# Xiaoming-Zhao/PointNav-VO

Hardware: AMD Instinct MI355X
Metric: RGB-D frame-pair VO inferences/s @341x192 (higher is better)
Workload: dtype f32

## Files before the change

pointnav-vo_amd/csrc/conv_x3.hip:

```cpp
#include <cmath>
#include <cstdio>
#include <cstdlib>
#include <cstring>

#include "pnvo_internal.h"

namespace pnvo {

typedef float f32x16 __attribute__((ext_vector_type(16)));
typedef float f32x4 __attribute__((ext_vector_type(4)));
typedef float f32x2 __attribute__((ext_vector_type(2)));
typedef __bf16 bf16x8 __attribute__((ext_vector_type(8)));
typedef __bf16 bf16x2 __attribute__((ext_vector_type(2)));
typedef _Float16 f16x8 __attribute__((ext_vector_type(8)));
typedef _Float16 f16x2 __attribute__((ext_vector_type(2)));
typedef unsigned u32x4 __attribute__((ext_vector_type(4)));

namespace {
__device__ __forceinline__ unsigned pack2(float a, float b) {
  const bf16x2 r = __builtin_convertvector(f32x2{a, b}, bf16x2);
  return __builtin_bit_cast(unsigned, r);
}
__device__ __forceinline__ unsigned pack2h(float a, float b) {
  const f16x2 r = __builtin_convertvector(f32x2{a, b}, f16x2);
  return __builtin_bit_cast(unsigned, r);
}
__device__ __forceinline__ float lo_f(unsigned u) { return __builtin_bit_cast(float, u << 16); }
__device__ __forceinline__ float hi_f(unsigned u) { return __builtin_bit_cast(float, u & 0xffff0000u); }
}

constexpr int x3_wpe(int mw, int nw, int np, bool dsf = false) {
  return dsf ? (mw * nw >= 6 ? 1 : (mw * nw >= 2 ? 2 : 3)) : ((np == 2 && mw * nw <= 2) ? 3 : 2);
}

template <int KS, int STRIDE, int MODE, int MW, int NW, int NP, bool DSF = false, bool W8 = false, bool KSW = false>
__global__ __launch_bounds__(W8 ? 512 : 256) __attribute__((amdgpu_waves_per_eu(W8 ? 2 : x3_wpe(MW, NW, NP, DSF), W8 ? 2 : x3_wpe(MW, NW, NP, DSF)))) void conv_x3_kernel(const ConvX3Args p) {
  constexpr int NTH = W8 ? 512 : 256, NWV = NTH / 64;
  constexpr int EMW = KSW ? 1 : MW;
  static_assert(!KSW || (NW == 1 && NP == 2 && KS == 3 && !DSF && !W8), "K split over the waves: float16-piece 3x3 convs, one N-tile");
  static_assert(!DSF || (KS == 3 && STRIDE == 2 && NP == 2 && (MODE == 0 || MODE == 2)), "the downsample rides on a float16-piece 3x3 stride-2 conv");
  extern __shared__ __attribute__((aligned(16))) unsigned char lds[];
  constexpr int PSTEP = KS == 1 ? STRIDE : 1;
  constexpr int CS = KS == 1 ? 1 : STRIDE;
  constexpr int PAD = KS / 2;
  const int lane = threadIdx.x & 63;
  const int wave = __builtin_amdgcn_readfirstlane(threadIdx.x >> 6);

  const int ntiles = p.B * p.tiles_r * p.tiles_c;
  const int chunk = (ntiles + 7) >> 3;
  int bid = (int)(blockIdx.x & 7) * chunk + (int)(blockIdx.x >> 3);
  if (bid >= ntiles) return;
  const int tci = bid % p.tiles_c;
  bid /= p.tiles_c;
  const int tri = bid % p.tiles_r;
  const int n = bid / p.tiles_r;
  const int r0 = tri * p.TR, c0 = tci * p.TC;
  const int hi0 = r0 * STRIDE - PAD, wi0 = c0 * STRIDE - PAD;
  const int mdl = (p.grp_end0 > 0 && n >= p.grp_end0) + (p.grp_end1 > 0 && n >= p.grp_end1);
  const unsigned short *g_wpk = mdl == 0 ? p.wpk : p.wpk_g[mdl - 1];
  const unsigned short *g_ds_wpk = mdl == 0 ? p.ds_wpk : p.ds_wpk_g[mdl - 1];
  const float g_oscale = mdl == 0 ? p.oscale : p.oscale_g[mdl - 1], g_ds_oscale = mdl == 0 ? p.ds_oscale : p.ds_oscale_g[mdl - 1];
  const float *g_gamma = mdl == 0 ? p.gn_gamma : p.gn_gamma_g[mdl - 1], *g_beta = mdl == 0 ? p.gn_beta : p.gn_beta_g[mdl - 1];
  const float *g_ds_gamma = mdl == 0 ? p.ds_gamma : p.ds_gamma_g[mdl - 1], *g_ds_beta = mdl == 0 ? p.ds_beta : p.ds_beta_g[mdl - 1];
  const int PR = p.PR, PC = p.PC, CK = p.CK;
  const int pitch = CK * 2 + 16;
  const int plane = PR * PC * pitch;
  const int npix = p.TR * p.TC;
  const int tab_off = KSW ? max(NP * plane, 4 * MW * 4096) : NP * plane;
  unsigned *qtab = reinterpret_cast<unsigned *>(lds + tab_off);
  unsigned *otab = qtab + p.MT * 32;
  for (int e = (int)threadIdx.x; e < p.MT * 32; e += NTH) {
    const int q = min(e, npix - 1);
    const int tr = q / p.TC, tc = q - tr * p.TC;
    qtab[e] = (unsigned)(((tr * CS) * PC + tc * CS) * pitch);
    const bool ok = e < npix && r0 + tr < p.Ho && c0 + tc < p.Wo;
    otab[e] = (unsigned)((tr * p.Wo + tc) * p.COUTP) | (ok ? 0u : 0x80000000u);
  }

  const int wn = p.wn;
  const int wave_m = wave / wn;
  const int wave_n = (wave & (wn - 1)) + (int)blockIdx.y * wn;
  const int ntt = p.COUTP >> 5, kct = p.CIN >> 4;

  f32x16 acc[MW][NW];
#pragma unroll
  for (int i = 0; i < MW; ++i)
#pragma unroll
    for (int j = 0; j < NW; ++j)
#pragma unroll
      for (int r = 0; r < 16; ++r) acc[i][j][r] = 0.f;
  f32x16 accd[DSF ? MW : 1][DSF ? NW : 1];
  if (DSF) {
#pragma unroll
    for (int i = 0; i < MW; ++i)
#pragma unroll
      for (int j = 0; j < NW; ++j)
#pragma unroll
        for (int r = 0; r < 16; ++r) accd[DSF ? i : 0][DSF ? j : 0][r] = 0.f;
  }

  float in_mul = 1.f, in_div = 1.f;
  const bool in_scaled = NP == 2 && p.in_absmax != nullptr;
  if (in_scaled) {
    unsigned mb = p.in_absmax[(threadIdx.x & 63) * 16];
#pragma unroll
    for (int d = 32; d >= 1; d >>= 1) mb = max(mb, (unsigned)__shfl_xor((int)mb, d));
    const int e = mb != 0u ? (int)((mb >> 23) & 0xffu) - 126 : 14;
    in_mul = __builtin_bit_cast(float, (unsigned)(14 - e + 127) << 23);
    in_div = __builtin_bit_cast(float, (unsigned)(e - 14 + 127) << 23);
  }
  const int G = CK >> 3;
  const int cg = threadIdx.x & (G - 1), pl = threadIdx.x / G, PS = NTH / G;
  const int dr = PS / PC, dc = PS - dr * PC;
  const int nppix = PR * PC;

  unsigned long long c_stage = 0, c_mm = 0, t_0 = __builtin_readcyclecounter(), r_0 = wall_clock64();
  for (int ck0 = 0; ck0 < p.CIN; ck0 += CK) {
    unsigned long long t_a = __builtin_readcyclecounter();
    if (ck0 > 0) __syncthreads();
    {
      f32x4 sc0, sc1, sh0, sh1, rs0, rs1, rt0, rt1;
      const bool res_ss = MODE == 2 && p.res_scale != nullptr;
      auto load_ss = [&]() {
        if (MODE >= 1) {
          const float *ps = p.in_scale + (long)n * p.CIN + ck0 + 8 * cg;
          const float *pt = p.in_shift + (long)n * p.CIN + ck0 + 8 * cg;
          sc0 = *reinterpret_cast<const f32x4 *>(ps);
          sc1 = *reinterpret_cast<const f32x4 *>(ps + 4);
          sh0 = *reinterpret_cast<const f32x4 *>(pt);
          sh1 = *reinterpret_cast<const f32x4 *>(pt + 4);
        }
        if (res_ss) {
          const float *ps = p.res_scale + (long)n * p.CIN + ck0 + 8 * cg;
          const float *pt = p.res_shift + (long)n * p.CIN + ck0 + 8 * cg;
          rs0 = *reinterpret_cast<const f32x4 *>(ps);
          rs1 = *reinterpret_cast<const f32x4 *>(ps + 4);
          rt0 = *reinterpret_cast<const f32x4 *>(pt);
          rt1 = *reinterpret_cast<const f32x4 *>(pt + 4);
        }
      };
      load_ss();
      int pr = pl / PC, pc = pl - pr * PC;
      const long img = ((long)n * p.H * p.W) * p.CIN + ck0 + 8 * cg;
      const float *xb = p.x + img;
      struct Round {
        f32x4 v[2][2], w[2][2];
        unsigned off[2];
        int gofs[2];
        bool ok[2], in[2], own[2];
      };
      auto fetch = [&](int pix, Round &r) {
#pragma unroll
        for (int k = 0; k < 2; ++k) {
          const int hi = hi0 + pr * PSTEP, wi = wi0 + pc * PSTEP;
          r.ok[k] = pix + k * PS < nppix;
          r.in[k] = r.ok[k] && hi >= 0 && hi < p.H && wi >= 0 && wi < p.W;
          r.off[k] = (unsigned)((pr * PC + pc) * pitch + 16 * cg);
          r.v[k][0] = r.v[k][1] = f32x4{0.f, 0.f, 0.f, 0.f};
          if (MODE >= 2) {
            r.own[k] = r.in[k] && p.xout != nullptr && blockIdx.y == 0 && pr >= PAD && pr < PAD + p.TR * CS && pc >= PAD && pc < PAD + p.TC * CS;
            r.gofs[k] = (hi * p.W + wi) * p.CIN;
          }
          if (r.in[k]) {
            const float *src = xb + ((long)hi * p.W + wi) * p.CIN;
            r.v[k][0] = *reinterpret_cast<const f32x4 *>(src);
            r.v[k][1] = *reinterpret_cast<const f32x4 *>(src + 4);
            if (MODE == 2) {
              const float *rsrc = p.res + img + ((long)hi * p.W + wi) * p.CIN;
              r.w[k][0] = *reinterpret_cast<const f32x4 *>(rsrc);
              r.w[k][1] = *reinterpret_cast<const f32x4 *>(rsrc + 4);
            }
          }
          pr += dr;
          pc += dc;
          if (pc >= PC) {
            pc -= PC;
            pr += 1;
          }
        }
      };
      auto split_store = [&](const Round &r) {
#pragma unroll
        for (int k = 0; k < 2; ++k) {
          if (!r.ok[k]) continue;
          float f[8];
#pragma unroll
          for (int e = 0; e < 8; ++e) {
            float t = r.v[k][e >> 2][e & 3];
            if (MODE == 1) {
              const f32x4 &sc = e < 4 ? sc0 : sc1, &sh = e < 4 ? sh0 : sh1;
              t = r.in[k] ? fmaxf(__builtin_fmaf(t, sc[e & 3], sh[e & 3]), 0.f) : 0.f;
            }
            if (MODE == 3) {
              const f32x4 &sc = e < 4 ? sc0 : sc1, &sh = e < 4 ? sh0 : sh1;
              int key = __builtin_bit_cast(int, t);
              key = key >= 0 ? key : key ^ 0x7fffffff;
              t = r.in[k] ? fmaxf(__builtin_fmaf(__builtin_bit_cast(float, key), __builtin_fabsf(sc[e & 3]), sh[e & 3]), 0.f) : 0.f;
            }
            if (MODE == 2) {
              const f32x4 &sc = e < 4 ? sc0 : sc1, &sh = e < 4 ? sh0 : sh1;
              float u = r.w[k][e >> 2][e & 3];
              if (res_ss) u = __builtin_fmaf(u, (e < 4 ? rs0 : rs1)[e & 3], (e < 4 ? rt0 : rt1)[e & 3]);
              t = r.in[k] ? fmaxf(__builtin_fmaf(t, sc[e & 3], sh[e & 3]) + u, 0.f) : 0.f;
            }
            f[e] = t;
          }
          if (MODE >= 2 && r.own[k]) {
            float *dst = p.xout + img + r.gofs[k];
            *reinterpret_cast<f32x4 *>(dst) = f32x4{f[0], f[1], f[2], f[3]};
            *reinterpret_cast<f32x4 *>(dst + 4) = f32x4{f[4], f[5], f[6], f[7]};
          }
          if (NP == 2) {
            if (in_scaled) {
#pragma unroll
              for (int e = 0; e < 8; ++e) f[e] *= in_mul;
            }
            u32x4 o0, o1;
#pragma unroll
            for (int e = 0; e < 4; ++e) {
              const float a = f[2 * e], b = f[2 * e + 1];
              const f16x2 h = __builtin_convertvector(f32x2{a, b}, f16x2);
              o0[e] = __builtin_bit_cast(unsigned, h);
              o1[e] = pack2h(a - (float)h[0], b - (float)h[1]);
            }
            *reinterpret_cast<u32x4 *>(lds + r.off[k]) = o0;
            *reinterpret_cast<u32x4 *>(lds + plane + r.off[k]) = o1;
            continue;
          }
          u32x4 o0, o1, o2;
#pragma unroll
          for (int e = 0; e < 4; ++e) {
            const float a = f[2 * e], b = f[2 * e + 1];
            const unsigned h = pack2(a, b);
            const float ra = a - lo_f(h), rb = b - hi_f(h);
            const unsigned m = pack2(ra, rb);
            o0[e] = h;
            o1[e] = m;
            o2[e] = pack2(ra - lo_f(m), rb - hi_f(m));
          }
          *reinterpret_cast<u32x4 *>(lds + r.off[k]) = o0;
          *reinterpret_cast<u32x4 *>(lds + plane + r.off[k]) = o1;
          *reinterpret_cast<u32x4 *>(lds + 2 * plane + r.off[k]) = o2;
        }
      };
      constexpr bool PIPE = !((MODE == 2 && (MW * NW >= 6 || x3_wpe(MW, NW, NP) == 3 || DSF)) || (DSF && MW * NW == 4));
      if (MW * NW <= 2 && !(MODE == 2 && (x3_wpe(MW, NW, NP) == 3 || DSF))) {
        for (int pix = pl; pix < nppix; pix += 6 * PS) {
          Round r0, r1, r2;
          fetch(pix, r0);
          fetch(pix + 2 * PS, r1);
          fetch(pix + 4 * PS, r2);
          split_store(r0);
          split_store(r1);
          split_store(r2);
        }
      } else if (PIPE) {
        Round cur, nxt;
        fetch(pl, cur);
        for (int pix = pl; pix < nppix; pix += 2 * PS) {
          const bool more = pix + 2 * PS < nppix;
          if (more) fetch(pix + 2 * PS, nxt);
          split_store(cur);
          if (more) cur = nxt;
        }
      } else {
        for (int pix = pl; pix < nppix; pix += 2 * PS) {
          Round cur;
          fetch(pix, cur);
          split_store(cur);
        }
      }
    }
    __syncthreads();
    unsigned long long t_b = __builtin_readcyclecounter();
    c_stage += t_b - t_a;

    unsigned aoff[MW];
#pragma unroll
    for (int i = 0; i < MW; ++i) {
      const int mt = min(KSW ? i : wave_m * MW + i, p.MT - 1);
      aoff[i] = qtab[mt * 32 + (lane & 31)] + (unsigned)((lane >> 5) * 16);
    }
    const int kcc = CK >> 4;
    const int nsteps = KS * KS * kcc;
    const unsigned kstep = (unsigned)ntt * (NP * 1024u);
    const char *wb_n = reinterpret_cast<const char *>(g_wpk) + (long)(ck0 >> 4) * kstep;
    unsigned toff_n = 0;
    int kc_n = 0, kw_n = 0;
    auto advance = [&]() {
      ++kc_n;
      toff_n += 32;
      wb_n += kstep;
      if (kc_n == kcc) {
        kc_n = 0;
        toff_n += (unsigned)(pitch - kcc * 32);
        wb_n += (long)(kct - kcc) * kstep;
        if (++kw_n == KS) {
          kw_n = 0;
          toff_n += (unsigned)((PC - KS) * pitch);
        }
      }
    };
    constexpr bool RING = NP == 2 && KS == 3 && MW * NW <= 2;
    const char *wb_b = wb_n;
    int kc_b = 0;
    auto advanceB = [&]() {
      wb_b += kstep;
      if (++kc_b == kcc) {
        kc_b = 0;
        wb_b += (long)(kct - kcc) * kstep;
      }
    };
    unsigned voff[NW];
#pragma unroll
    for (int j = 0; j < NW; ++j) voff[j] = (unsigned)min(wave_n * NW + j, ntt - 1) * (NP * 1024u) + (unsigned)lane * 16u;
    auto loadBr = [&](u32x4 (*b)[NW]) {
#pragma unroll
      for (int j = 0; j < NW; ++j)
#pragma unroll
        for (int pc = 0; pc < NP; ++pc) b[pc][j] = *reinterpret_cast<const u32x4 *>(wb_b + (size_t)voff[j] + pc * 1024);
    };
    auto loadA = [&](int i, u32x4 (*a)[MW]) {
#pragma unroll
      for (int pc = 0; pc < NP; ++pc) a[pc][i] = *reinterpret_cast<const u32x4 *>(lds + pc * plane + aoff[i] + toff_n);
    };
    auto loadB = [&](u32x4 (*b)[NW]) {
#pragma unroll
      for (int j = 0; j < NW; ++j)
#pragma unroll
        for (int pc = 0; pc < NP; ++pc) b[pc][j] = *reinterpret_cast<const u32x4 *>(wb_n + (size_t)voff[j] + pc * 1024);
    };
    auto step = [&](u32x4 (*a)[MW], const u32x4 (*b)[NW]) {
#pragma unroll
      for (int i = 0; i < MW; ++i) {
#pragma unroll
        for (int j = 0; j < NW; ++j) {
          if (NP == 2) {
            constexpr int TA[3] = {1, 0, 0}, TB[3] = {0, 1, 0};
#pragma unroll
            for (int t = 0; t < 3; ++t)
              acc[i][j] = __builtin_amdgcn_mfma_f32_32x32x16_f16(__builtin_bit_cast(f16x8, a[TA[t]][i]),
                                                                 __builtin_bit_cast(f16x8, b[TB[t]][j]), acc[i][j], 0, 0, 0);
          } else {
            constexpr int TA[6] = {1, 2, 0, 1, 0, 0}, TB[6] = {1, 0, 2, 0, 1, 0};
#pragma unroll
            for (int t = 0; t < 6; ++t)
              acc[i][j] = __builtin_amdgcn_mfma_f32_32x32x16_bf16(__builtin_bit_cast(bf16x8, a[TA[t]][i]),
                                                                  __builtin_bit_cast(bf16x8, b[TB[t]][j]), acc[i][j], 0, 0, 0);
          }
        }
        __builtin_amdgcn_sched_barrier(0);
        loadA(i, a);
        __builtin_amdgcn_sched_barrier(0);
      }
    };
    u32x4 a[NP][MW], b0[NP][NW], b1[NP][NW];
    u32x4 bd0[DSF ? NP : 1][NW], bd1[DSF ? NP : 1][NW];
    auto loadBd = [&](u32x4 (*b)[NW], int kc) {
      const char *wd = reinterpret_cast<const char *>(g_ds_wpk) + (long)((ck0 >> 4) + kc) * kstep;
#pragma unroll
      for (int j = 0; j < NW; ++j)
#pragma unroll
        for (int pc = 0; pc < NP; ++pc) b[pc][j] = *reinterpret_cast<const u32x4 *>(wd + (size_t)voff[j] + pc * 1024);
    };
    if constexpr (KSW) {
      const int s0 = (wave * nsteps) >> 2, s1 = ((wave + 1) * nsteps) >> 2;
      {
        const int tap = s0 / kcc, kc = s0 - tap * kcc, kh = tap / KS, kw = tap - kh * KS;
        kc_n = kc;
        kw_n = kw;
        toff_n = (unsigned)((kh * PC + kw) * pitch + kc * 32);
        wb_n += ((long)tap * kct + kc) * kstep;
        kc_b = kc;
        wb_b = wb_n;
      }
      u32x4 br[3][NP][NW];
      int fb = s0;
      auto fetchB = [&](u32x4 (*bq)[NW]) {
        loadBr(bq);
        if (++fb < s1) advanceB();
      };
      fetchB(br[0]);
      fetchB(br[1]);
#pragma unroll
      for (int i = 0; i < MW; ++i) loadA(i, a);
      if (s0 + 1 < s1) advance();
#pragma unroll 1
      for (int s = s0; s < s1; s += 3) {
#pragma unroll
        for (int u = 0; u < 3; ++u) {
          if (s + u >= s1) break;
          fetchB(br[(u + 2) % 3]);
          __builtin_amdgcn_sched_barrier(0);
          step(a, br[u]);
          if (s + u + 2 < s1) advance();
        }
      }
    } else {
    if (DSF) loadBd(bd0, 0);
    loadB(b0);
#pragma unroll
    for (int i = 0; i < MW; ++i) loadA(i, a);
    advance();
    if (RING) {
      constexpr int R = MW * NW <= 2 ? 6 : 3;
      u32x4 br[R][NP][NW];
#pragma unroll
      for (int pc = 0; pc < NP; ++pc)
#pragma unroll
        for (int j = 0; j < NW; ++j) br[0][pc][j] = b0[pc][j];
#pragma unroll
      for (int q = 1; q < R - 1; ++q) {
        advanceB();
        loadBr(br[q]);
      }
      advanceB();
      constexpr bool A2 = MW * NW <= 2 && !(MODE == 2 && MW * NW == 2 && !DSF) && !(MODE == 2 && DSF && MW * NW == 1);
      u32x4 a1[A2 ? NP : 1][MW];
      if (A2) {
#pragma unroll
        for (int i = 0; i < MW; ++i) loadA(i, a1);
        advance();
      }
#pragma unroll 1
      for (int s = 0; s < nsteps; s += R) {
#pragma unroll
        for (int u = 0; u < R; ++u) {
          loadBr(br[(u + R - 1) % R]);
          if (s + u + R < nsteps) advanceB();
          __builtin_amdgcn_sched_barrier(0);
          if (A2) {
            step((u & 1) ? a1 : a, br[u]);
            if (s + u + 3 < nsteps) advance();
          } else {
            step(a, br[u]);
            if (s + u + 2 < nsteps) advance();
          }
        }
      }
    } else {
#pragma unroll 1
      for (int s = 0; s < nsteps; s += 2) {
        const bool more = s + 2 < nsteps;
        loadB(b1);
        __builtin_amdgcn_sched_barrier(0);
        step(a, b0);
        if (more) advance();
        loadB(b0);
        __builtin_amdgcn_sched_barrier(0);
        step(a, b1);
        if (more) advance();
      }
    }
    }
    if constexpr (DSF) {
      const unsigned tc0 = (unsigned)((PC + 1) * pitch);
      u32x4 ad[NP][MW];
      auto loadAd = [&](int kc) {
#pragma unroll
        for (int i = 0; i < MW; ++i)
#pragma unroll
          for (int pc = 0; pc < NP; ++pc) ad[pc][i] = *reinterpret_cast<const u32x4 *>(lds + pc * plane + aoff[i] + tc0 + (unsigned)kc * 32u);
      };
      auto mm = [&](const u32x4 (*bd)[NW]) {
        constexpr int TA[3] = {1, 0, 0}, TB[3] = {0, 1, 0};
#pragma unroll
        for (int i = 0; i < MW; ++i)
#pragma unroll
          for (int j = 0; j < NW; ++j)
#pragma unroll
            for (int t = 0; t < 3; ++t)
              accd[i][j] = __builtin_amdgcn_mfma_f32_32x32x16_f16(__builtin_bit_cast(f16x8, ad[TA[t]][i]), __builtin_bit_cast(f16x8, bd[TB[t]][j]),
                                                                  accd[i][j], 0, 0, 0);
      };
      if constexpr (MW * NW == 4) {
#pragma unroll 1
        for (int kc = 0; kc < kcc; ++kc) {
          loadAd(kc);
          mm(bd0);
          if (kc + 1 < kcc) loadBd(bd0, kc + 1);
        }
      } else {
#pragma unroll 1
        for (int kc = 0; kc < kcc; kc += 2) {
          loadAd(kc);
          loadBd(bd1, kc + 1);
          mm(bd0);
          loadAd(kc + 1);
          if (kc + 2 < kcc) loadBd(bd0, kc + 2);
          mm(bd1);
        }
      }
    }
    c_mm += __builtin_readcyclecounter() - t_b;
  }
  if constexpr (KSW) {
    __syncthreads();
    float *part = reinterpret_cast<float *>(lds);
#pragma unroll
    for (int i = 0; i < MW; ++i)
#pragma unroll
      for (int r = 0; r < 16; ++r) part[((wave * MW + i) * 16 + r) * 64 + lane] = acc[i][0][r];
    __syncthreads();
    const int mt = min(wave, MW - 1);
#pragma unroll
    for (int r = 0; r < 16; ++r) {
      float v = part[((0 * MW + mt) * 16 + r) * 64 + lane];
#pragma unroll
      for (int w = 1; w < 4; ++w) v += part[((w * MW + mt) * 16 + r) * 64 + lane];
      acc[0][0][r] = v;
    }
    __syncthreads();
  }
  unsigned long long t_e = __builtin_readcyclecounter();

  const int rr16 = lane >> 5;
  const long ybase = (((long)n * p.Ho + r0) * p.Wo + c0) * p.COUTP;
  auto emit = [&](f32x16 (*ac)[NW], float *yout, float *stats, const float *oscale_ptr, float oscale, const float *gamma, const float *beta,
                  float *gscale, float *gshift, float *gmu, float *grstd, bool again) {
    if (NP == 2) {
      const float os = (oscale_ptr != nullptr ? *oscale_ptr : oscale) * in_div;
#pragma unroll
      for (int i = 0; i < EMW; ++i)
#pragma unroll
        for (int j = 0; j < NW; ++j)
#pragma unroll
          for (int r = 0; r < 16; ++r) ac[i][j][r] *= os;
    }
    float t1[NW], t2[NW];
#pragma unroll
    for (int j = 0; j < NW; ++j) t1[j] = t2[j] = 0.f;
#pragma unroll
    for (int i = 0; i < EMW; ++i) {
      const int mt = KSW ? wave : wave_m * MW + i;
      if (mt >= p.MT) continue;
      u32x4 ent[4];
#pragma unroll
      for (int g4 = 0; g4 < 4; ++g4) ent[g4] = *reinterpret_cast<const u32x4 *>(otab + mt * 32 + 8 * g4 + 4 * rr16);
      unsigned flags = 0;
#pragma unroll
      for (int g4 = 0; g4 < 4; ++g4) flags |= ent[g4][0] | ent[g4][1] | ent[g4][2] | ent[g4][3];
      const bool whole = !__any((int)(flags >> 31));
#pragma unroll
      for (int j = 0; j < NW; ++j) {
        const int nt = wave_n * NW + j;
        if (nt >= ntt) continue;
        const int co = nt * 32 + (lane & 31);
        float s1 = 0.f, s2 = 0.f;
        if (whole) {
#pragma unroll
          for (int r = 0; r < 16; ++r) {
            const float v = ac[i][j][r];
            (yout + ybase + co)[ent[r >> 2][r & 3]] = v;
            s1 += v;
            s2 = __builtin_fmaf(v, v, s2);
          }
        } else {
#pragma unroll
          for (int r = 0; r < 16; ++r) {
            const unsigned e = ent[r >> 2][r & 3];
            const bool ok = (int)e >= 0;
            const float v = ok ? ac[i][j][r] : 0.f;
            if (ok) (yout + ybase + co)[e] = v;
            s1 += v;
            s2 = __builtin_fmaf(v, v, s2);
          }
        }
        t1[j] += s1 + __shfl_xor(s1, 32);
        t2[j] += s2 + __shfl_xor(s2, 32);
      }
    }
    if (stats != nullptr) {
// ... 200 lines not shown
  fetch(cur);
  for (int vb = (int)blockIdx.x;; vb += (int)gridDim.x) {
    if ((int)threadIdx.x < p.MT * 32) {
      const int q = min((int)threadIdx.x, npix - 1);
      const int tr = q / p.TC, tc = q - tr * p.TC;
      const bool ok = (int)threadIdx.x < npix && cur.r0 + tr < p.Ho && cur.c0 + tc < p.Wo;
      otab[threadIdx.x] = (unsigned)((tr * p.Wo + tc) * p.COUTP) | (ok ? 0u : 0x80000000u);
    }
    split_store(cur);
    __syncthreads();
    const Tile nxt = decode(vb + (int)gridDim.x);
    if (!BRES && nxt.valid) fetch(nxt);

    f32x16 acc[MW][NW];
#pragma unroll
    for (int i = 0; i < MW; ++i)
#pragma unroll
      for (int j = 0; j < NW; ++j)
#pragma unroll
        for (int r = 0; r < 16; ++r) acc[i][j][r] = 0.f;
    unsigned aoff[MW];
#pragma unroll
    for (int i = 0; i < MW; ++i) {
      const int mt = min(wave_m * MW + i, p.MT - 1);
      aoff[i] = qtab[mt * 32 + (lane & 31)] + (unsigned)((lane >> 5) * 16);
    }
    const int kcc = CK >> 4;
    const int nsteps = KS * KS * kcc;
    const unsigned kstep = (unsigned)ntt * (NP * 1024u);
    const char *wb_n = reinterpret_cast<const char *>(p.wpk);
    unsigned toff_n = 0;
    int kc_n = 0, kw_n = 0;
    auto advance = [&]() {
      ++kc_n;
      toff_n += 32;
      wb_n += kstep;
      if (kc_n == kcc) {
        kc_n = 0;
        toff_n += (unsigned)(pitch - kcc * 32);
        if (++kw_n == KS) {
          kw_n = 0;
          toff_n += (unsigned)((PC - KS) * pitch);
        }
      }
    };
    unsigned voff[NW];
#pragma unroll
    for (int j = 0; j < NW; ++j) voff[j] = (unsigned)min(wave_n * NW + j, ntt - 1) * (NP * 1024u) + (unsigned)lane * 16u;
    auto loadA = [&](int i, u32x4 (*a)[MW]) {
#pragma unroll
      for (int pc = 0; pc < NP; ++pc) a[pc][i] = *reinterpret_cast<const u32x4 *>(lds + pc * plane + aoff[i] + toff_n);
    };
    auto loadB = [&](u32x4 (*b)[NW]) {
#pragma unroll
      for (int j = 0; j < NW; ++j)
#pragma unroll
        for (int pc = 0; pc < NP; ++pc) b[pc][j] = *reinterpret_cast<const u32x4 *>(wb_n + (size_t)voff[j] + pc * 1024);
    };
    auto step = [&](u32x4 (*a)[MW], const u32x4 (*b)[NW]) {
#pragma unroll
      for (int i = 0; i < MW; ++i) {
#pragma unroll
        for (int j = 0; j < NW; ++j) {
          constexpr int TA[3] = {1, 0, 0}, TB[3] = {0, 1, 0};
#pragma unroll
          for (int t = 0; t < 3; ++t)
            acc[i][j] = __builtin_amdgcn_mfma_f32_32x32x16_f16(__builtin_bit_cast(f16x8, a[TA[t]][i]),
                                                               __builtin_bit_cast(f16x8, b[TB[t]][j]), acc[i][j], 0, 0, 0);
        }
        __builtin_amdgcn_sched_barrier(0);
        loadA(i, a);
        __builtin_amdgcn_sched_barrier(0);
      }
    };
    u32x4 a[NP][MW], b0[NP][NW], b1[NP][NW];
    if (BRES) {
#pragma unroll
      for (int i = 0; i < MW; ++i) loadA(i, a);
#pragma unroll
      for (int st = 0; st < 18; ++st) {
        const int nx = st + 1, ntap = nx >> 1, nkc = nx & 1;
        toff_n = (unsigned)(((ntap / 3) * PC + (ntap % 3)) * pitch + nkc * 32);
        if (st == 17) toff_n = 0;
#pragma unroll
        for (int i = 0; i < MW; ++i) {
          constexpr int TA[3] = {1, 0, 0}, TB[3] = {0, 1, 0};
#pragma unroll
          for (int t = 0; t < 3; ++t)
            acc[i][0] = __builtin_amdgcn_mfma_f32_32x32x16_f16(__builtin_bit_cast(f16x8, a[TA[t]][i]),
                                                               __builtin_bit_cast(f16x8, bres[BRES ? st : 0][TB[t]]), acc[i][0], 0, 0, 0);
          __builtin_amdgcn_sched_barrier(0);
          loadA(i, a);
          __builtin_amdgcn_sched_barrier(0);
        }
      }
    } else {
      loadB(b0);
#pragma unroll
      for (int i = 0; i < MW; ++i) loadA(i, a);
      advance();
#pragma unroll 1
      for (int s = 0; s < nsteps; s += 2) {
        const bool more = s + 2 < nsteps;
        loadB(b1);
        __builtin_amdgcn_sched_barrier(0);
        step(a, b0);
        if (more) advance();
        loadB(b0);
        __builtin_amdgcn_sched_barrier(0);
        step(a, b1);
        if (more) advance();
      }
    }

    {
      const float os = (p.oscale_ptr != nullptr ? *p.oscale_ptr : p.oscale) * in_div;
#pragma unroll
      for (int i = 0; i < MW; ++i)
#pragma unroll
        for (int j = 0; j < NW; ++j)
#pragma unroll
          for (int r = 0; r < 16; ++r) acc[i][j][r] *= os;
    }
    const int rr16 = lane >> 5;
    const long ybase = (((long)cur.n * p.Ho + cur.r0) * p.Wo + cur.c0) * p.COUTP;
    float t1[NW], t2[NW];
#pragma unroll
    for (int j = 0; j < NW; ++j) t1[j] = t2[j] = 0.f;
#pragma unroll
    for (int i = 0; i < MW; ++i) {
      const int mt = wave_m * MW + i;
      if (mt >= p.MT) continue;
      u32x4 ent[4];
#pragma unroll
      for (int g4 = 0; g4 < 4; ++g4) ent[g4] = *reinterpret_cast<const u32x4 *>(otab + mt * 32 + 8 * g4 + 4 * rr16);
      unsigned flags = 0;
#pragma unroll
      for (int g4 = 0; g4 < 4; ++g4) flags |= ent[g4][0] | ent[g4][1] | ent[g4][2] | ent[g4][3];
      const bool whole = !__any((int)(flags >> 31));
#pragma unroll
      for (int j = 0; j < NW; ++j) {
        const int nt = wave_n * NW + j;
        if (nt >= ntt) continue;
        const int co = nt * 32 + (lane & 31);
        float s1 = 0.f, s2 = 0.f;
        if (whole) {
#pragma unroll
          for (int r = 0; r < 16; ++r) {
            const float x = acc[i][j][r];
            (p.y + ybase + co)[ent[r >> 2][r & 3]] = x;
            s1 += x;
            s2 = __builtin_fmaf(x, x, s2);
          }
        } else {
#pragma unroll
          for (int r = 0; r < 16; ++r) {
            const unsigned e = ent[r >> 2][r & 3];
            const bool ok = (int)e >= 0;
            const float x = ok ? acc[i][j][r] : 0.f;
            if (ok) (p.y + ybase + co)[e] = x;
            s1 += x;
            s2 = __builtin_fmaf(x, x, s2);
          }
        }
        t1[j] += s1 + __shfl_xor(s1, 32);
        t2[j] += s2 + __shfl_xor(s2, 32);
      }
    }
    if (p.stats != nullptr) {
      const int rows = 4 / wn;
      float *red = reinterpret_cast<float *>(lds);
      if (rows > 1) {
        __syncthreads();
        if (lane < 32)
#pragma unroll
          for (int j = 0; j < NW; ++j) *reinterpret_cast<f32x2 *>(red + ((wave * NW + j) * 32 + lane) * 2) = f32x2{t1[j], t2[j]};
        __syncthreads();
      }
      if (wave_m == 0 && lane < 32) {
#pragma unroll
        for (int j = 0; j < NW; ++j) {
          const int nt = wave_n * NW + j;
          if (nt >= ntt) continue;
          float s1 = t1[j], s2 = t2[j];
          for (int w = 1; w < rows; ++w) {
            const f32x2 o = *reinterpret_cast<const f32x2 *>(red + (((w * wn + (wave & (wn - 1))) * NW + j) * 32 + lane) * 2);
            s1 += o[0];
            s2 += o[1];
          }
          float *dst = p.stats + (((long)cur.n * p.slots + cur.tri * p.tiles_c + cur.tci) * p.COUTP + nt * 32 + lane) * 2;
          dst[0] = s1;
          dst[1] = s2;
        }
      }
    }
    if (!nxt.valid) break;
    if (BRES) fetch(nxt);
    __syncthreads();
    cur = nxt;
  }
}

namespace {
template <int KS, int STRIDE, int NP>
hipError_t launch_ks(const ConvX3Args &a, int mode, int mw, int nw, dim3 grid, size_t ldsb, hipStream_t s) {
#define PNVO_X3(MODE_, MW_, NW_)                                                                          \
  if (mode == MODE_ && mw == MW_ && nw == NW_) {                                                          \
    hipLaunchKernelGGL((conv_x3_kernel<KS, STRIDE, MODE_, MW_, NW_, NP>), grid, dim3(256), ldsb, s, a);   \
    return hipGetLastError();                                                                             \
  }
  if constexpr (KS == 3 && STRIDE == 2 && NP == 2) {
    if (a.ds_wpk != nullptr) {
#define PNVO_X3D(MODE_, MW_, NW_)                                                                               \
  if (mode == MODE_ && mw == MW_ && nw == NW_) {                                                                \
    hipLaunchKernelGGL((conv_x3_kernel<KS, STRIDE, MODE_, MW_, NW_, NP, true>), grid, dim3(256), ldsb, s, a);   \
    return hipGetLastError();                                                                                   \
  }
      if (a.w8) {
#define PNVO_X3DW(MODE_)                                                                                                  \
  if (mode == MODE_ && mw == 3 && nw == 1) {                                                                             \
    hipLaunchKernelGGL((conv_x3_kernel<KS, STRIDE, MODE_, 3, 1, NP, true, true>), grid, dim3(512), ldsb, s, a);          \
    return hipGetLastError();                                                                                            \
  }
        PNVO_X3DW(0) PNVO_X3DW(2)
#undef PNVO_X3DW
        return hipErrorInvalidValue;
      }
      PNVO_X3D(0, 1, 1) PNVO_X3D(2, 1, 1) PNVO_X3D(0, 2, 1) PNVO_X3D(2, 2, 1) PNVO_X3D(0, 2, 2) PNVO_X3D(2, 2, 2) PNVO_X3D(0, 3, 2) PNVO_X3D(2, 3, 2)
#undef PNVO_X3D
      return hipErrorInvalidValue;
    }
  }
  PNVO_X3(0, 1, 1) PNVO_X3(1, 1, 1) PNVO_X3(0, 2, 1) PNVO_X3(1, 2, 1) PNVO_X3(0, 2, 2) PNVO_X3(1, 2, 2) PNVO_X3(0, 3, 2) PNVO_X3(1, 3, 2)
  PNVO_X3(2, 1, 1) PNVO_X3(2, 2, 1) PNVO_X3(2, 2, 2) PNVO_X3(2, 3, 2) PNVO_X3(3, 1, 1) PNVO_X3(3, 2, 1) PNVO_X3(3, 2, 2) PNVO_X3(3, 3, 2)

  if (KS == 3 && STRIDE == 1 && NP == 2) {
    PNVO_X3(0, 5, 1) PNVO_X3(1, 5, 1) PNVO_X3(2, 5, 1) PNVO_X3(3, 5, 1)
    if constexpr (KS == 3 && STRIDE == 1 && NP == 2) if (a.ksw) {
#define PNVO_X3K(MODE_, MW_)                                                                                             \
  if (mode == MODE_ && mw == MW_ && nw == 1) {                                                                          \
    hipLaunchKernelGGL((conv_x3_kernel<KS, STRIDE, MODE_, MW_, 1, NP, false, false, true>), grid, dim3(256), ldsb, s, a); \
    return hipGetLastError();                                                                                           \
  }
      PNVO_X3K(0, 3) PNVO_X3K(1, 3) PNVO_X3K(2, 3) PNVO_X3K(0, 4) PNVO_X3K(1, 4) PNVO_X3K(2, 4)
#undef PNVO_X3K
      return hipErrorInvalidValue;
    }
  }
  if constexpr (KS == 3 && NP == 2) if (a.w8) {
#define PNVO_X3W(MODE_)                                                                                                  \
  if (mode == MODE_ && mw == 3 && nw == 1) {                                                                            \
  hipLaunchKernelGGL((conv_x3_kernel<KS, STRIDE, MODE_, 3, 1, NP, false, true>), grid, dim3(512), ldsb, s, a);        \
  return hipGetLastError();                                                                                           \
  }
    PNVO_X3W(0) PNVO_X3W(1) PNVO_X3W(2) PNVO_X3W(3)
#undef PNVO_X3W
    return hipErrorInvalidValue;
  }
#undef PNVO_X3
  return hipErrorInvalidValue;
}
}

namespace {
bool conv_x3_plan_impl(ConvX3Args &a, int ks, int stride, int *mw, int *nw, size_t *lds_bytes, bool fine);
long plan_wgs(const ConvX3Args &a, int nw) {
  const int ntt = a.COUTP / 32;
  return (long)a.B * a.tiles_r * a.tiles_c * ((ntt + a.wn * nw - 1) / (a.wn * nw));
}
}

bool conv_x3_plan(ConvX3Args &a, int ks, int stride, int *mw, int *nw, size_t *lds_bytes) {
  ConvX3Args reg = a;
  int rmw = 0, rnw = 0;
  size_t rlds = 0;
  const int force0 = a.force;
  reg.force = 1;
  const bool reg_ok = conv_x3_plan_impl(reg, ks, stride, &rmw, &rnw, &rlds, false);
  const long reg_wgs = reg_ok ? plan_wgs(reg, rnw) : 0;
  const int ntt = a.COUTP / 32;
  if (a.fine && a.np == 2 && ntt >= 2 && (!reg_ok || reg_wgs < 224)) {
    ConvX3Args f = a;
    int fmw = 0, fnw = 0;
    size_t flds = 0;
    f.force = 1;
    if (conv_x3_plan_impl(f, ks, stride, &fmw, &fnw, &flds, true)) {
      const long fw = plan_wgs(f, fnw);
      if (fw > reg_wgs && (fw >= 48 || force0)) {
        f.force = force0;
        a = f;
        *mw = fmw;
        *nw = fnw;
        *lds_bytes = flds;
        return true;
      }
    }
  }
  return conv_x3_plan_impl(a, ks, stride, mw, nw, lds_bytes, false);
}

namespace {
bool conv_x3_plan_impl(ConvX3Args &a, int ks, int stride, int *mw, int *nw, size_t *lds_bytes, bool fine) {
  if (a.CIN % 32 || a.COUTP % 32 || a.COUTP > 1024 || a.CIN > 1024) return false;
  if (!((ks == 3 && (stride == 1 || stride == 2)) || (ks == 1 && stride == 2))) return false;
  a.w8 = 0;
  a.ksw = 0;
  const int ntt = a.COUTP / 32;
  int TR, TC;
  if (stride == 2 && ks == 3) {
    TC = a.Wo >= 32 ? 16 : a.Wo;
    const int pc = 2 * TC + 1;
    TR = (324 / pc - 1) / 2;
    if (TR < 1) return false;
    if (TR > a.Ho) TR = a.Ho;
    while (TR > 1 && TR * TC > (ntt == 2 ? 64 : (ntt == 4 ? 128 : 96))) --TR;
  } else if (ntt == 1 && stride == 1 && ks == 3 && a.CIN > 32 && a.np == 2 && a.Wo < 32 && a.Ho * a.Wo <= 128) {
    TC = a.Wo;
    TR = a.Ho;
  } else if (ntt == 1) {
    if (stride != 1 || ks != 3 || a.CIN != 32) return false;
    TC = a.Wo >= 16 ? 16 : a.Wo;
    TR = 256 / TC;
    while (TR > 1 && (TR + 2) * (TC + 2) > 324) --TR;
    if (TR > a.Ho) TR = a.Ho;
    if (TR * TC <= 96) return false;
  } else if (a.strip && !fine && a.np == 2 && stride == 1 && ks == 3 && ntt == 4 && a.Wo >= 16 && a.Ho >= 8) {
    const int ncol = (a.Wo + 21) / 22;
    TC = (a.Wo + ncol - 1) / ncol;
    TR = 288 / TC;
    if (TR > a.Ho) TR = a.Ho;
    const int nrow = (a.Ho + TR - 1) / TR;
    TR = (a.Ho + nrow - 1) / nrow;
  } else if (a.Wo >= 32) {
    TR = 8;
    TC = 16;
  } else {
    TC = a.Wo;
    int target = ntt == 4 ? 192 : (ntt >= 8 ? 96 : 128);
    if (fine && a.ksw_ok && ks == 3 && stride == 1 && a.np == 2 && a.CIN >= 128) target = 96;
    TR = target / TC;
    if (TR < 1) TR = 1;
    if (TR > a.Ho) TR = a.Ho;
  }
  a.TR = TR;
  a.TC = TC;
  a.tiles_r = (a.Ho + TR - 1) / TR;
  a.tiles_c = (a.Wo + TC - 1) / TC;
  a.MT = (TR * TC + 31) / 32;
  const int cs = ks == 1 ? 1 : stride;
  a.PR = (TR - 1) * cs + ks;
  a.PC = (TC - 1) * cs + ks;
  const bool strip = a.strip && !fine && a.np == 2 && stride == 1 && ks == 3 && ntt == 4 && a.Wo >= 16 && a.Ho >= 8 && a.MT > 6;
  if (fine) {
    if (a.MT > 8) return false;
    a.wn = 1;
    *mw = (a.MT + 3) / 4;
    *nw = 1;
    if (a.ksw_ok && (a.MT == 3 || a.MT == 4) && ks == 3 && stride == 1 && a.np == 2 && a.CIN >= 128) {
      a.ksw = 1;
      *mw = a.MT;
    }
  } else if (strip) {
    a.wn = 2;
    *mw = (a.MT + 1) / 2;
    *nw = 1;
    if (*mw > 5) return false;
    if (*mw < 5) *mw = 5;
  } else if (ntt == 1) {
    a.wn = 1;
    *mw = a.CIN > 32 ? 1 : 2;
    *nw = 1;
    if (a.ksw_ok && a.CIN >= 128 && (a.MT == 3 || a.MT == 4) && ks == 3 && stride == 1 && a.np == 2) {
      a.ksw = 1;
      *mw = a.MT;
    }
  } else if (ntt == 2) {
    a.wn = 2;
    *mw = a.MT > 2 ? 2 : 1;
    *nw = 1;
  } else if (ntt == 4) {
    a.wn = 2;
    *mw = a.MT > 4 ? 3 : 2;
    *nw = 2;
  } else {
    a.wn = 4;
    *mw = a.MT > 2 ? 3 : 2;
    *nw = 2;
    const long ntiles = (long)a.B * a.tiles_r * a.tiles_c;
    if (ntiles < 200 && a.MT <= 4) {
      a.wn = 2;
      *mw = 2;
    }
    if (a.w8_ok && !fine && ntiles >= 200 && a.MT == 3 && ntt == 8 && a.np == 2 && ks == 3) {
      a.w8 = 1;
      a.wn = 8;
      *mw = 3;
      *nw = 1;
    }
  }
  if (!a.ksw && ((a.w8 ? 8 : 4) / a.wn) * *mw < a.MT) return false;
  const size_t np = a.np == 2 ? 2 : 3;
  int ck = 32;
  while (ck < 256 && a.CIN % (2 * ck) == 0) ck *= 2;
  const size_t cap = (size_t)72 * 1024;
  while (ck > 32 && np * a.PR * a.PC * (ck * 2 + 16) > cap) ck /= 2;
  if (np * a.PR * a.PC * (ck * 2 + 16) > cap + 4096) return false;
  if (a.CIN % ck) return false;
  a.CK = ck;
  {
    const bool force = a.force != 0;
    const long wgs = (long)a.B * a.tiles_r * a.tiles_c * ((ntt + a.wn * *nw - 1) / (a.wn * *nw));
    if (wgs < (a.np == 2 ? 112 : 192) && !force) return false;
  }
  a.slots = a.tiles_r * a.tiles_c;
  *lds_bytes = np * a.PR * a.PC * (ck * 2 + 16) + (size_t)a.MT * 32 * 4 * 2;
  if (a.ksw) *lds_bytes = std::max(np * a.PR * a.PC * (ck * 2 + 16), (size_t)4 * a.MT * 4096) + (size_t)a.MT * 32 * 4 * 2;
  return true;
}
}

bool conv_x3_persistent(const ConvX3Args &a, int ks, int stride, int mode, int mw, int nw) {
  const long ntiles = (long)a.B * a.tiles_r * a.tiles_c;
  const int ntt = a.COUTP / 32, pwgs = a.persist_wgs;
  const bool bres = ntt == 1 && a.CIN == 32 && nw == 1 && (mode == 0 || mode == 1);
  return a.np == 2 && ks == 3 && stride == 1 && bres && mw * nw <= 2 && a.CK == a.CIN && pwgs >= 8 &&
         (long)a.PR * a.PC * (a.CK / 8) <= 6 * 256 && ntiles >= 2L * pwgs;
}

hipError_t launch_conv_x3(const ConvX3Args &a0, int ks, int stride, int mode, int mw, int nw, size_t lds_bytes, hipStream_t s) {
  ConvX3Args a = a0;
  static unsigned long long *prof = nullptr;
  static const bool want = std::getenv("PNVO_X3_PROF") != nullptr;
  if (want && !prof) {
    (void)hipMalloc((void **)&prof, 512);
    (void)hipMemset(prof, 0, 512);
  }
  a.prof = prof;
  struct Dump {
    const ConvX3Args &a; int mw, nw; hipStream_t s; unsigned long long *prof;
    ~Dump() {
      static int calls = 0;
      if (!prof || ++calls > 40) return;
      unsigned long long h[64];
      (void)hipStreamSynchronize(s);
      (void)hipMemcpy(h, prof, 512, hipMemcpyDeviceToHost);
      std::fprintf(stderr, "[pnvo] conv_x3 B %d %dx%d cin %d cout %d tile %dx%d MT %d CK %d (%d,%d) wn %d: wave0 stage %llu mfma %llu epi %llu total %llu "
                           "(100MHz ticks %llu) | wave3 stage %llu mfma %llu epi %llu total %llu\n", a.B, a.Ho, a.Wo, a.CIN, a.COUTP, a.TR, a.TC,
                   a.MT, a.CK, mw, nw, a.wn, h[0], h[1], h[2], h[3], h[4], h[24], h[25], h[26], h[27]);
    }
  } dump{a, mw, nw, s, prof};
  const long ntiles = (long)a.B * a.tiles_r * a.tiles_c;
  const int ntt = a.COUTP / 32, per_wg = a.wn * nw;
  dim3 grid((unsigned)(((ntiles + 7) / 8) * 8), (unsigned)((ntt + per_wg - 1) / per_wg), 1u);
  const int pwgs = a.persist_wgs;
  if (conv_x3_persistent(a, ks, stride, mode, mw, nw)) {
    const bool bres = true;
    dim3 pg((unsigned)(pwgs & ~7), grid.y, 1u);
    if (bres) pg.x = (unsigned)(((pwgs / 3) * 2) & ~7);
#define PNVO_X3P(MODE_, MW_, NW_)                                                                        \
  if (mode == MODE_ && mw == MW_ && nw == NW_) {                                                         \
    hipLaunchKernelGGL((conv_x3p_kernel<MODE_, MW_, NW_, true>), pg, dim3(256), lds_bytes, s, a);       \
    return hipGetLastError();                                                                            \
  }
    PNVO_X3P(0, 1, 1) PNVO_X3P(1, 1, 1) PNVO_X3P(0, 2, 1) PNVO_X3P(1, 2, 1)
#undef PNVO_X3P
  }
  if (a.np == 2) {
    if (ks == 3 && stride == 1) return launch_ks<3, 1, 2>(a, mode, mw, nw, grid, lds_bytes, s);
    if (ks == 3 && stride == 2) return launch_ks<3, 2, 2>(a, mode, mw, nw, grid, lds_bytes, s);
    if (ks == 1 && stride == 2) return launch_ks<1, 2, 2>(a, mode, mw, nw, grid, lds_bytes, s);
    return hipErrorInvalidValue;
  }
  if (ks == 3 && stride == 1) return launch_ks<3, 1, 3>(a, mode, mw, nw, grid, lds_bytes, s);
  if (ks == 3 && stride == 2) return launch_ks<3, 2, 3>(a, mode, mw, nw, grid, lds_bytes, s);
  if (ks == 1 && stride == 2) return launch_ks<1, 2, 3>(a, mode, mw, nw, grid, lds_bytes, s);
  return hipErrorInvalidValue;
}

void pack_conv_x3_weight(const float *oihw, int cout, int cin, int cinp, int coutp, int kh_, int kw_, unsigned short *out) {
  const int T = kh_ * kw_, kct = cinp / 16, ntt = coutp / 32;
  auto bf = [](float f) {
    unsigned u;
    std::memcpy(&u, &f, 4);
    if ((u & 0x7f800000u) == 0x7f800000u) return (unsigned short)(u >> 16);
    u += 0x7fffu + ((u >> 16) & 1u);
    return (unsigned short)(u >> 16);
  };
  auto tof = [](unsigned short h) {
    const unsigned u = (unsigned)h << 16;
    float f;
    std::memcpy(&f, &u, 4);
    return f;
  };
  for (int tap = 0; tap < T; ++tap)
    for (int kc = 0; kc < kct; ++kc)
      for (int nt = 0; nt < ntt; ++nt)
        for (int ln = 0; ln < 64; ++ln)
          for (int j = 0; j < 8; ++j) {
            const int co = nt * 32 + (ln & 31), ci = 16 * kc + 8 * (ln >> 5) + j;
            float v = 0.f;
            if (co < cout && ci < cin) v = oihw[((size_t)co * cin + ci) * T + tap];
            const unsigned short h = bf(v);
            const float r1 = v - tof(h);
            const unsigned short m = bf(r1);
            const unsigned short l = bf(r1 - tof(m));
            const size_t base = ((((size_t)tap * kct + kc) * ntt + nt) * 3) * 64 * 8 + (size_t)ln * 8 + j;
            out[base] = h;
            out[base + 64 * 8] = m;
            out[base + 2 * 64 * 8] = l;
          }
}

static unsigned short f32_to_f16_rne(float f) {
  const _Float16 h = (_Float16)f;
  unsigned short u;
  std::memcpy(&u, &h, 2);
  return u;
}
static float f16_to_f32(unsigned short u) {
  _Float16 h;
  std::memcpy(&h, &u, 2);
  return (float)h;
}
float pack_conv_x2_weight(const float *oihw, int cout, int cin, int cinp, int coutp, int kh_, int kw_, unsigned short *out) {
  const int T = kh_ * kw_, kct = cinp / 16, ntt = coutp / 32;
  float mx = 0.f;
  for (size_t k = 0; k < (size_t)cout * cin * T; ++k) mx = std::fmax(mx, std::fabs(oihw[k]));
  int e = 0;
  if (mx > 0.f) std::frexp(mx, &e);
  const float scale = std::ldexp(1.0f, 12 - e), inv = std::ldexp(1.0f, e - 12);
  for (int tap = 0; tap < T; ++tap)
    for (int kc = 0; kc < kct; ++kc)
      for (int nt = 0; nt < ntt; ++nt)
        for (int ln = 0; ln < 64; ++ln)
          for (int j = 0; j < 8; ++j) {
            const int co = nt * 32 + (ln & 31), ci = 16 * kc + 8 * (ln >> 5) + j;
            float v = 0.f;
            if (co < cout && ci < cin) v = oihw[((size_t)co * cin + ci) * T + tap] * scale;
            const unsigned short h = f32_to_f16_rne(v);
            const unsigned short m = f32_to_f16_rne(v - f16_to_f32(h));
            const size_t base = ((((size_t)tap * kct + kc) * ntt + nt) * 2) * 64 * 8 + (size_t)ln * 8 + j;
            out[base] = h;
            out[base + 64 * 8] = m;
          }
  return inv;
}

__global__ __launch_bounds__(256) void conv_x3_repack_kernel(const float *w, int cout, int cin, int cinp, int coutp, int T,
                                                           int transposed, unsigned short *out, long total) {
  const long e = (long)blockIdx.x * 256 + threadIdx.x;
  if (e >= total) return;
  const int j = (int)(e & 7), ln = (int)((e >> 3) & 63);
  long r = e >> 9;
  const int ntt = coutp / 32, kct = cinp / 16;
  const int nt = (int)(r % ntt);
  r /= ntt;
  const int kc = (int)(r % kct), tap = (int)(r / kct);
  const int co = nt * 32 + (ln & 31), ci = 16 * kc + 8 * (ln >> 5) + j;
  const float v = (co < cout && ci < cin) ? (transposed ? w[((long)ci * cout + co) * T + (T - 1 - tap)] : w[((long)co * cin + ci) * T + tap])
                                          : 0.f;
  const unsigned h = pack2(v, 0.f) & 0xffffu;
  const float r1 = v - lo_f(h);
  const unsigned m = pack2(r1, 0.f) & 0xffffu;
  const unsigned l = pack2(r1 - lo_f(m), 0.f) & 0xffffu;
  const long base = ((((long)tap * kct + kc) * ntt + nt) * 3) * 512 + (long)ln * 8 + j;
  out[base] = (unsigned short)h;
  out[base + 512] = (unsigned short)m;
  out[base + 1024] = (unsigned short)l;
}

constexpr int X2_SCALE_CHUNKS = 32;
__global__ __launch_bounds__(256) void conv_x2_absmax_kernel(const float *params, const long *seg, unsigned *bits) {
  const long off = seg[2 * blockIdx.x], n = seg[2 * blockIdx.x + 1];
  const long per = (n + X2_SCALE_CHUNKS - 1) / X2_SCALE_CHUNKS;
  const long lo = per * blockIdx.y, hi = lo + per < n ? lo + per : n;
  float mx = 0.f;
  for (long i = lo + threadIdx.x; i < hi; i += 1024) {
    const float a = fabsf(params[off + i]);
    const float b = i + 256 < hi ? fabsf(params[off + i + 256]) : 0.f;
    const float c = i + 512 < hi ? fabsf(params[off + i + 512]) : 0.f;
    const float d = i + 768 < hi ? fabsf(params[off + i + 768]) : 0.f;
    mx = fmaxf(fmaxf(mx, fmaxf(a, b)), fmaxf(c, d));
  }
#pragma unroll
  for (int d = 32; d >= 1; d >>= 1) mx = fmaxf(mx, __shfl_xor(mx, d));
  if ((threadIdx.x & 63) == 0 && mx > 0.f) atomicMax(&bits[blockIdx.x], __builtin_bit_cast(unsigned, mx));
}

__global__ __launch_bounds__(256) void conv_x2_scale_finish_kernel(unsigned *bits, float *out, int nseg) {
  const int k = blockIdx.x * 256 + threadIdx.x;
  if (k >= nseg) return;
  const unsigned mb = bits[k];
  bits[k] = 0u;
  int e = 0;
  if (mb != 0u) e = (int)((mb >> 23) & 0xffu) - 126;
  out[2 * k] = __builtin_bit_cast(float, (unsigned)(12 - e + 127) << 23);
  out[2 * k + 1] = __builtin_bit_cast(float, (unsigned)(e - 12 + 127) << 23);
}

hipError_t launch_conv_x2_scales(const float *params, const long *seg_dev, int nseg, float *out, hipStream_t s) {
  if (nseg <= 0) return hipSuccess;
  unsigned *bits = reinterpret_cast<unsigned *>(out + 2 * nseg);
  hipLaunchKernelGGL(conv_x2_absmax_kernel, dim3((unsigned)nseg, X2_SCALE_CHUNKS), dim3(256), 0, s, params, seg_dev, bits);
  hipLaunchKernelGGL(conv_x2_scale_finish_kernel, dim3((unsigned)((nseg + 255) / 256)), dim3(256), 0, s, bits, out, nseg);
  return hipGetLastError();
}
// ... 39 lines not shown
```

Baseline: 112,700.

## Use buffer loads with OOB masking and software-pipelined staging in conv_x3

Replaces the guarded global loads and stores in the input-staging loop with raw buffer loads and stores. These use a per-image resource descriptor, and an out-of-range offset (0x80000000) stands in for branches on boundary and padding pixels, since out-of-range accesses return zero or are dropped. The staging loop is restructured around per-pixel records with sched_barriers. It batches 6 fetches ahead in the small-wave case and ping-pongs two records in all other cases, which also enables prefetching for configurations that were previously unpipelined. A planner guard rejects images whose byte size would overflow the 32-bit buffer offset. The aim is fewer branches, less address arithmetic and more loads in flight, at the cost of higher register pressure.

```diff
diff --git a/pointnav-vo_amd/csrc/conv_x3.hip b/pointnav-vo_amd/csrc/conv_x3.hip
--- a/pointnav-vo_amd/csrc/conv_x3.hip
+++ b/pointnav-vo_amd/csrc/conv_x3.hip
@@ -141,133 +141,124 @@
       };
       load_ss();
       int pr = pl / PC, pc = pl - pr * PC;
-      const long img = ((long)n * p.H * p.W) * p.CIN + ck0 + 8 * cg;
-      const float *xb = p.x + img;
-      struct Round {
-        f32x4 v[2][2], w[2][2];
-        unsigned off[2];
-        int gofs[2];
-        bool ok[2], in[2], own[2];
+      constexpr unsigned OOB = 0x80000000u;
+      const long sbase = ((long)n * p.H * p.W) * p.CIN;
+      const unsigned sbytes = (unsigned)(p.H * p.W * p.CIN) * 4u;
+      auto rsrc = [&](const float *t) {
+        return __builtin_amdgcn_make_buffer_rsrc(const_cast<float *>(t != nullptr ? t + sbase : p.x), 0, t != nullptr ? sbytes : 0u, 0x00020000);
       };
-      auto fetch = [&](int pix, Round &r) {
-#pragma unroll
-        for (int k = 0; k < 2; ++k) {
-          const int hi = hi0 + pr * PSTEP, wi = wi0 + pc * PSTEP;
-          r.ok[k] = pix + k * PS < nppix;
-          r.in[k] = r.ok[k] && hi >= 0 && hi < p.H && wi >= 0 && wi < p.W;
-          r.off[k] = (unsigned)((pr * PC + pc) * pitch + 16 * cg);
-          r.v[k][0] = r.v[k][1] = f32x4{0.f, 0.f, 0.f, 0.f};
-          if (MODE >= 2) {
-            r.own[k] = r.in[k] && p.xout != nullptr && blockIdx.y == 0 && pr >= PAD && pr < PAD + p.TR * CS && pc >= PAD && pc < PAD + p.TC * CS;
-            r.gofs[k] = (hi * p.W + wi) * p.CIN;
-          }
-          if (r.in[k]) {
-            const float *src = xb + ((long)hi * p.W + wi) * p.CIN;
-            r.v[k][0] = *reinterpret_cast<const f32x4 *>(src);
-            r.v[k][1] = *reinterpret_cast<const f32x4 *>(src + 4);
-            if (MODE == 2) {
-              const float *rsrc = p.res + img + ((long)hi * p.W + wi) * p.CIN;
-              r.w[k][0] = *reinterpret_cast<const f32x4 *>(rsrc);
-              r.w[k][1] = *reinterpret_cast<const f32x4 *>(rsrc + 4);
-            }
-          }
-          pr += dr;
-          pc += dc;
-          if (pc >= PC) {
-            pc -= PC;
-            pr += 1;
-          }
-        }
+      const __amdgpu_buffer_rsrc_t rx = rsrc(p.x), rres = rsrc(MODE == 2 ? p.res : nullptr), rxo = rsrc(MODE >= 2 ? p.xout : nullptr);
+      const unsigned cb = (unsigned)(ck0 + 8 * cg) * 4u;
+      const unsigned own_en = (MODE >= 2 && p.xout != nullptr && blockIdx.y == 0) ? 1u : 0u;
+      const unsigned own_r = (unsigned)(p.TR * CS), own_c = (unsigned)(p.TC * CS);
+      struct Px {
+        f32x4 v[2], w[2];
+        unsigned m;
       };
-      auto split_store = [&](const Round &r) {
-#pragma unroll
-        for (int k = 0; k < 2; ++k) {
-          if (!r.ok[k]) continue;
-          float f[8];
-#pragma unroll
-          for (int e = 0; e < 8; ++e) {
-            float t = r.v[k][e >> 2][e & 3];
-            if (MODE == 1) {
-              const f32x4 &sc = e < 4 ? sc0 : sc1, &sh = e < 4 ? sh0 : sh1;
-              t = r.in[k] ? fmaxf(__builtin_fmaf(t, sc[e & 3], sh[e & 3]), 0.f) : 0.f;
-            }
-            if (MODE == 3) {
-              const f32x4 &sc = e < 4 ? sc0 : sc1, &sh = e < 4 ? sh0 : sh1;
-              int key = __builtin_bit_cast(int, t);
-              key = key >= 0 ? key : key ^ 0x7fffffff;
-              t = r.in[k] ? fmaxf(__builtin_fmaf(__builtin_bit_cast(float, key), __builtin_fabsf(sc[e & 3]), sh[e & 3]), 0.f) : 0.f;
-            }
-            if (MODE == 2) {
-              const f32x4 &sc = e < 4 ? sc0 : sc1, &sh = e < 4 ? sh0 : sh1;
-              float u = r.w[k][e >> 2][e & 3];
-              if (res_ss) u = __builtin_fmaf(u, (e < 4 ? rs0 : rs1)[e & 3], (e < 4 ? rt0 : rt1)[e & 3]);
-              t = r.in[k] ? fmaxf(__builtin_fmaf(t, sc[e & 3], sh[e & 3]) + u, 0.f) : 0.f;
-            }
-            f[e] = t;
-          }
-          if (MODE >= 2 && r.own[k]) {
-            float *dst = p.xout + img + r.gofs[k];
-            *reinterpret_cast<f32x4 *>(dst) = f32x4{f[0], f[1], f[2], f[3]};
-            *reinterpret_cast<f32x4 *>(dst + 4) = f32x4{f[4], f[5], f[6], f[7]};
-          }
-          if (NP == 2) {
-            if (in_scaled) {
-#pragma unroll
-              for (int e = 0; e < 8; ++e) f[e] *= in_mul;
-            }
-            u32x4 o0, o1;
-#pragma unroll
-            for (int e = 0; e < 4; ++e) {
-              const float a = f[2 * e], b = f[2 * e + 1];
-              const f16x2 h = __builtin_convertvector(f32x2{a, b}, f16x2);
-              o0[e] = __builtin_bit_cast(unsigned, h);
-              o1[e] = pack2h(a - (float)h[0], b - (float)h[1]);
-            }
-            *reinterpret_cast<u32x4 *>(lds + r.off[k]) = o0;
-            *reinterpret_cast<u32x4 *>(lds + plane + r.off[k]) = o1;
-            continue;
-          }
-          u32x4 o0, o1, o2;
+      auto fetch = [&](int pix, Px &q) {
+        const int hi = hi0 + pr * PSTEP, wi = wi0 + pc * PSTEP;
+        const unsigned in = (unsigned)(pix < nppix) & (unsigned)((unsigned)hi < (unsigned)p.H) & (unsigned)((unsigned)wi < (unsigned)p.W);
+        unsigned e = (unsigned)((hi * p.W + wi) * p.CIN) * 4u + cb;
+        asm volatile("" : "+v"(e));
+        const unsigned vo = in ? e : OOB;
+        q.v[0] = __builtin_bit_cast(f32x4, __builtin_amdgcn_raw_buffer_load_b128(rx, vo, 0, 0));
+        q.v[1] = __builtin_bit_cast(f32x4, __builtin_amdgcn_raw_buffer_load_b128(rx, vo + 16u, 0, 0));
+        if (MODE == 2) {
+          q.w[0] = __builtin_bit_cast(f32x4, __builtin_amdgcn_raw_buffer_load_b128(rres, vo, 0, 0));
+          q.w[1] = __builtin_bit_cast(f32x4, __builtin_amdgcn_raw_buffer_load_b128(rres, vo + 16u, 0, 0));
+        }
+        unsigned own = 0u;
+        if (MODE >= 2) own = in & own_en & (unsigned)((unsigned)(pr - PAD) < own_r) & (unsigned)((unsigned)(pc - PAD) < own_c);
+        q.m = vo | own;
+        pr += dr;
+        pc += dc;
+        const int carry = pc >= PC ? 1 : 0;
+        pc -= carry * PC;
+        pr += carry;
+      };
+      auto split_store = [&](int pix, const Px &q) {
+        const bool in = (int)q.m >= 0;
+        float f[8];
+#pragma unroll
+        for (int e = 0; e < 8; ++e) {
+          float t = q.v[e >> 2][e & 3];
+          if (MODE == 1) {
+            const f32x4 &sc = e < 4 ? sc0 : sc1, &sh = e < 4 ? sh0 : sh1;
+            t = in ? fmaxf(__builtin_fmaf(t, sc[e & 3], sh[e & 3]), 0.f) : 0.f;
+          }
+          if (MODE == 3) {
+            const f32x4 &sc = e < 4 ? sc0 : sc1, &sh = e < 4 ? sh0 : sh1;
+            int key = __builtin_bit_cast(int, t);
+            key = key >= 0 ? key : key ^ 0x7fffffff;
+            t = in ? fmaxf(__builtin_fmaf(__builtin_bit_cast(float, key), __builtin_fabsf(sc[e & 3]), sh[e & 3]), 0.f) : 0.f;
+          }
+          if (MODE == 2) {
+            const f32x4 &sc = e < 4 ? sc0 : sc1, &sh = e < 4 ? sh0 : sh1;
+            float u = q.w[e >> 2][e & 3];
+            if (res_ss) u = __builtin_fmaf(u, (e < 4 ? rs0 : rs1)[e & 3], (e < 4 ? rt0 : rt1)[e & 3]);
+            t = in ? fmaxf(__builtin_fmaf(t, sc[e & 3], sh[e & 3]) + u, 0.f) : 0.f;
+          }
+          f[e] = t;
+        }
+        if (MODE >= 2) {
+          const unsigned so = (q.m & 1u) ? (q.m & ~1u) : OOB;
+          __builtin_amdgcn_raw_buffer_store_b128(__builtin_bit_cast(u32x4, f32x4{f[0], f[1], f[2], f[3]}), rxo, so, 0, 0);
+          __builtin_amdgcn_raw_buffer_store_b128(__builtin_bit_cast(u32x4, f32x4{f[4], f[5], f[6], f[7]}), rxo, so + 16u, 0, 0);
+        }
+        const unsigned off = pix < nppix ? (unsigned)(pix * pitch + 16 * cg) : (unsigned)(CK * 2);
+        if (NP == 2) {
+          if (in_scaled) {
+#pragma unroll
+            for (int e = 0; e < 8; ++e) f[e] *= in_mul;
+          }
+          u32x4 o0, o1;
 #pragma unroll
           for (int e = 0; e < 4; ++e) {
             const float a = f[2 * e], b = f[2 * e + 1];
-            const unsigned h = pack2(a, b);
-            const float ra = a - lo_f(h), rb = b - hi_f(h);
-            const unsigned m = pack2(ra, rb);
-            o0[e] = h;
-            o1[e] = m;
-            o2[e] = pack2(ra - lo_f(m), rb - hi_f(m));
-          }
-          *reinterpret_cast<u32x4 *>(lds + r.off[k]) = o0;
-          *reinterpret_cast<u32x4 *>(lds + plane + r.off[k]) = o1;
-          *reinterpret_cast<u32x4 *>(lds + 2 * plane + r.off[k]) = o2;
-        }
+            const f16x2 h = __builtin_convertvector(f32x2{a, b}, f16x2);
+            o0[e] = __builtin_bit_cast(unsigned, h);
+            o1[e] = pack2h(a - (float)h[0], b - (float)h[1]);
+          }
+          *reinterpret_cast<u32x4 *>(lds + off) = o0;
+          *reinterpret_cast<u32x4 *>(lds + plane + off) = o1;
+          return;
+        }
+        u32x4 o0, o1, o2;
+#pragma unroll
+        for (int e = 0; e < 4; ++e) {
+          const float a = f[2 * e], b = f[2 * e + 1];
+          const unsigned h = pack2(a, b);
+          const float ra = a - lo_f(h), rb = b - hi_f(h);
+          const unsigned m = pack2(ra, rb);
+          o0[e] = h;
+          o1[e] = m;
+          o2[e] = pack2(ra - lo_f(m), rb - hi_f(m));
+        }
+        *reinterpret_cast<u32x4 *>(lds + off) = o0;
+        *reinterpret_cast<u32x4 *>(lds + plane + off) = o1;
+        *reinterpret_cast<u32x4 *>(lds + 2 * plane + off) = o2;
       };
-      constexpr bool PIPE = !((MODE == 2 && (MW * NW >= 6 || x3_wpe(MW, NW, NP) == 3 || DSF)) || (DSF && MW * NW == 4));
+      const int nrounds = (nppix + PS - 1) / PS;
       if (MW * NW <= 2 && !(MODE == 2 && (x3_wpe(MW, NW, NP) == 3 || DSF))) {
-        for (int pix = pl; pix < nppix; pix += 6 * PS) {
-          Round r0, r1, r2;
-          fetch(pix, r0);
-          fetch(pix + 2 * PS, r1);
-          fetch(pix + 4 * PS, r2);
-          split_store(r0);
-          split_store(r1);
-          split_store(r2);
-        }
-      } else if (PIPE) {
-        Round cur, nxt;
-        fetch(pl, cur);
-        for (int pix = pl; pix < nppix; pix += 2 * PS) {
-          const bool more = pix + 2 * PS < nppix;
-          if (more) fetch(pix + 2 * PS, nxt);
-          split_store(cur);
-          if (more) cur = nxt;
+        for (int r = 0; r < nrounds; r += 6) {
+          Px q[6];
+#pragma unroll
+          for (int k = 0; k < 6; ++k) fetch(pl + (r + k) * PS, q[k]);
+          __builtin_amdgcn_sched_barrier(0);
+#pragma unroll
+          for (int k = 0; k < 6; ++k) split_store(pl + (r + k) * PS, q[k]);
         }
       } else {
-        for (int pix = pl; pix < nppix; pix += 2 * PS) {
-          Round cur;
-          fetch(pix, cur);
-          split_store(cur);
+        Px qa, qb;
+        fetch(pl, qa);
+        for (int r = 0; r < nrounds; r += 2) {
+          fetch(pl + (r + 1) * PS, qb);
+          __builtin_amdgcn_sched_barrier(0);
+          split_store(pl + r * PS, qa);
+          if (r + 1 >= nrounds) break;
+          fetch(pl + (r + 2) * PS, qa);
+          __builtin_amdgcn_sched_barrier(0);
+          split_store(pl + (r + 1) * PS, qb);
         }
       }
     }
@@ -1074,6 +1065,7 @@
 namespace {
 bool conv_x3_plan_impl(ConvX3Args &a, int ks, int stride, int *mw, int *nw, size_t *lds_bytes, bool fine) {
   if (a.CIN % 32 || a.COUTP % 32 || a.COUTP > 1024 || a.CIN > 1024) return false;
+  if ((long)a.H * a.W * a.CIN * 4 >= (1L << 31)) return false;
   if (!((ks == 3 && (stride == 1 || stride == 2)) || (ks == 1 && stride == 2))) return false;
   a.w8 = 0;
   a.ksw = 0;
```

Result: no change. 113,300 (median of 6 runs) (+0.5%).
